# yuw444/fastF

Hardware: AMD Instinct MI355X
Metric: BAM records/sec -> deduped UMI matrix; achieved HBM GB/s vs roofline (higher is better)
Workload: dtype u64

## Files before the change

fastf_amd/csrc/umi_engine.hip:

```cpp
#include "umi_kernels.hpp"
#include "sweep_kernels.hpp"
#include "cap_kernels.hpp"
#include "level_kernels.hpp"
#include "gene_kernels.hpp"
#include "cells_kernels.hpp"
#include "fidelity_kernels.hpp"
#include "gene_fidelity_kernels.hpp"
#include "neighbors_kernels.hpp"
#include "labels_kernels.hpp"

#include <algorithm>
#include <cstdarg>
#include <cstdio>
#include <cstdlib>
#include <cstring>
#include <mutex>
#include <new>
#include <stdexcept>
#include <chrono>
#include <string>
#include <thread>
#include <utility>
#include <vector>

// ... 210 lines not shown
    bool h_coo_pinned = false; u32 h_coo_uses = 0;
    u32* lent_rows = nullptr; u64 lent_cap = 0;
    u32* rows_at = nullptr; u64 rows_stride = 0;
    std::vector<u32> h_ufeature, h_ucell, h_uumi, h_ncopy;
    std::vector<uint8_t> h_unonnull;
    u64 total_records = 0, hits_so_far = 0, keys_so_far = 0;
    u64 c_sampled = 0, c_valid = 0;
    bool finished = false; int sorted_in_tmp = 0; u64 n_sorted = 0;
    u32 skip_bits = 0;
    bool fully_sorted = false;
    DevBuf d_cellidx, d_tilecnt, d_tilebase, d_binbase, d_cnt;
    DevBuf d_halfhits;
    DevBuf d_segkeys;
    DevBuf d_segcount, d_segprefix, d_tileseg;
    u32 giant_parity = 0;
    u32 seg_n = 0; u64 seg_stride = 0;
    DevBuf d_rgn_phys, d_rgn_hist, d_rgn_blk;
    u32 rgn_hist_n = 0, rgn_hist_shift = 0;
    bool stream_mode = false, store_regions = false;
    bool stream_single = false, stream_sharded = false, stream_off = false;
    bool narrow = false, genes_one_family = false;
    u64 slots_used = 0, slot_cap = 0; u32 rgn_n = 0, rgn_cap = 0;
    DevBuf d_scanblk;
    DevBuf d_rg_feature, d_rg_cell, d_rg_count, d_rg_ukeys, d_spanrows, d_spanbase, d_giant;
    u32 rg_n = 0; bool rg_umi = false;
    bool wide = false, long_umi = false; u32 group_bits = 0;
    u32 sub_bits = 0, row_split = 0;
    bool finish_queued = false;
    DevBuf d_vals, d_vtmp;
    bool timing = false;
    hipEvent_t t_ev[2] = {nullptr, nullptr};
    double t_scatter_ms = 0; u64 t_scatter_n = 0;
    double t_k1_ms = 0; u64 t_k1_n = 0;
    double t_k1b_ms = 0; u64 t_k1b_n = 0;
    double t_k3_ms = 0; u64 t_k3_n = 0;
    double t_count_ms = 0; u64 t_count_n = 0;
    double t_gather_ms = 0; u64 t_gather_n = 0;
};
// ... 344 lines not shown
    (void)hipDeviceSynchronize();
    for (int i = 0; i < 2; ++i) {
        fastf_engine::Slot& sl = e->slot[i];
        if (sl.h_stage) (void)hipHostFree(sl.h_stage);
        if (sl.h_draws) (void)hipHostFree(sl.h_draws);
        if (sl.h_small) (void)hipHostFree(sl.h_small);
        sl.d_stage.release();
        if (sl.ev_copy) (void)hipEventDestroy(sl.ev_copy);
        if (sl.ev_done) (void)hipEventDestroy(sl.ev_done);
        if (e->t_ev[i]) (void)hipEventDestroy(e->t_ev[i]);
    }
    if (e->h_small) (void)hipHostFree(e->h_small);
    if (e->h_coo) { if (e->h_coo_pinned) pin_unreg(e->h_coo); fastf_big_free(e->h_coo, (size_t)e->h_coo_cap * 12); }
    e->d_ring.release(); e->d_mt.release(); e->d_nbr.release(); e->d_dbits.release(); e->d_mtwords.release(); e->d_mtsub.release(); e->d_mtpoly.release(); e->d_mtseat.release(); e->d_mtseq.release();
    DevBuf* all[] = {&e->tab_cells, &e->tab_feats, &e->img_cells, &e->img_genes, &e->d_cell_filter, &e->d_keys, &e->d_tmp, &e->d_small, &e->d_feature, &e->d_cell,
                     &e->d_count, &e->d_ukeys, &e->d_ncopy, &e->d_cellidx, &e->d_tilecnt, &e->d_tilebase, &e->d_binbase, &e->d_cnt, &e->d_rg_feature, &e->d_rg_cell, &e->d_rg_count, &e->d_rg_ukeys, &e->d_spanrows, &e->d_spanbase, &e->d_giant, &e->d_scanblk,
                     &e->d_halfhits, &e->d_segcount, &e->d_segprefix, &e->d_tileseg, &e->d_segkeys, &e->d_vals, &e->d_vtmp,
                     &e->d_rgn_phys, &e->d_rgn_hist, &e->d_rgn_blk};
    for (DevBuf* b : all) b->release();
    if (e->s_compute) (void)hipStreamDestroy(e->s_compute);
    if (e->s_copy) (void)hipStreamDestroy(e->s_copy);
    if (e->s_mt) (void)hipStreamDestroy(e->s_mt);
    if (e->ev_mt) (void)hipEventDestroy(e->ev_mt);
    delete e;
} FASTF_CATCH_VOID

extern "C" int fastf_engine_table_modes(const fastf_engine_t* e, int* cells_in_lds, int* genes_in_lds) FASTF_TRY {
    if (!e) return set_err("null engine");
    if (cells_in_lds) *cells_in_lds = e->use_lds_cells;
    if (genes_in_lds) *genes_in_lds = e->use_lds_genes ? (e->lds_genes.direct ? 2 : 1) : 0;
    return 0;
} FASTF_CATCH_INT

// ... 83 lines not shown
    e->t_scatter_n = e->t_k1_n = e->t_k1b_n = e->t_k3_n = e->t_count_n = e->t_gather_n = 0;
    return 0;
} FASTF_CATCH_INT
extern "C" int fastf_engine_get_timing(fastf_engine_t* e, int which, double* total_ms, uint64_t* launches) FASTF_TRY {
    if (!e) return set_err("null engine");
    const double ms[6] = {e->t_k1_ms, e->t_scatter_ms, e->t_k3_ms, e->t_count_ms, e->t_k1b_ms, e->t_gather_ms};
    const u64 n[6] = {e->t_k1_n, e->t_scatter_n, e->t_k3_n, e->t_count_n, e->t_k1b_n, e->t_gather_n};
    if (which < 0 || which > 5) return set_err("bad timer index");
    *total_ms = ms[which]; *launches = n[which];
    return 0;
} FASTF_CATCH_INT

static u64* g_k1_stamps = nullptr;
extern "C" void fastf_debug_set_k1_stamps(void* p) { g_k1_stamps = (u64*)p; }

static void launch_scan_tiles(fastf_engine* e, int slot, hipStream_t s, u32* in, u64* out, u32 T, u64* total_out, u64* running, u64* base_out) {
    constexpr u32 CHUNK = 16u * 1024u;
    const u32 n_blk = (T + CHUNK - 1) / CHUNK;
    if (n_blk <= 1 || n_blk > 64 || e->d_scanblk.ensure(2 * 64 * sizeof(u64))) {
        hipLaunchKernelGGL(scan_tiles_kernel<16>, dim3(1), dim3(1024), 0, s, in, out, T, total_out, running, base_out, (u64*)nullptr);
        return;
    }
    u64* const blk = (u64*)e->d_scanblk.p + 64 * slot;
    hipLaunchKernelGGL(scan_tiles_kernel<16>, dim3(n_blk), dim3(1024), 0, s, in, out, T, (u64*)nullptr, (u64*)nullptr, (u64*)nullptr, blk);
    hipLaunchKernelGGL(scan_fix_kernel<16>, dim3(n_blk), dim3(1024), 0, s, out, T, (const u64*)blk, n_blk, total_out, running, base_out);
}

static int launch_probe_cells(fastf_engine* e, const u64* cb, u64 n, u64* d_total_out, hipStream_t s,
                              u64* d_running = nullptr, u64* d_base_out = nullptr, void* blk = nullptr) {
    if (reserve_workspace(e, blk ? 0 : n, 0, n)) return 1;
    const u32 tiles = (u32)((n + K1_TILE - 1) / K1_TILE);
    const CellOut cout = blk ? CellOut{blk, blk_run_bytes(e->cell16, e->narrow), blk_cell_off(e->narrow)} : CellOut{e->d_cellidx.p, 0u, 0u};
    t_begin(e, s);
    if (e->use_lds_cells) {
        const u32 grid = std::min<u32>(e->cells_blocks_per_cu * g_cu_count, (tiles + 1) / 2);
        if (e->cells_blocks_per_cu >= 2)
            hipLaunchKernelGGL(probe_cells_lds_kernel<true>, dim3(grid), dim3(1024), e->lds_cells.bytes, s, cb, n, e->lds_cells,
                               cout, e->cell16, (u32*)e->d_tilecnt.p, (u32*)e->d_halfhits.p, tiles);
        else
            hipLaunchKernelGGL(probe_cells_lds_kernel<false>, dim3(grid), dim3(1024), e->lds_cells.bytes, s, cb, n, e->lds_cells,
                               cout, e->cell16, (u32*)e->d_tilecnt.p, (u32*)e->d_halfhits.p, tiles);
    } else if (e->cell_filter.bits) {
        const u32 grid = std::min<u32>(tiles, 4 * g_cu_count);
        hipLaunchKernelGGL(probe_cells_filtered_kernel, dim3(grid), dim3(K1_THREADS), (e->cell_filter.mask + 1u) / 8u, s, cb, n,
                           e->cells, e->cell_filter, cout, e->cell16, (u32*)e->d_tilecnt.p, (u32*)e->d_halfhits.p, tiles);
    } else {
        hipLaunchKernelGGL(probe_cells_kernel<0>, dim3(tiles), dim3(K1_THREADS), 0, s, cb, n, e->cells,
                           cout, e->cell16, (u32*)e->d_tilecnt.p, (u32*)e->d_halfhits.p);
    }
    t_end(e, s, &e->t_k1_ms, &e->t_k1_n);
    dbg_sync(s, "K1a probe_cells");
    launch_scan_tiles(e, 0, s, (u32*)e->d_tilecnt.p, (u64*)e->d_tilebase.p, tiles, d_total_out, d_running, d_base_out);
    dbg_sync(s, "K1a tile scan");
    HIP_OK(hipGetLastError());
    return 0;
}

extern "C" int fastf_dev_count_hits(fastf_engine_t* e, const uint64_t* d_cb_key, uint64_t n,
                                    uint64_t* d_hits_out, void* stream) FASTF_TRY {
    DEV_ENTRY(!e, "null engine");
    hipStream_t s = (hipStream_t)stream;
    if (n == 0) { HIP_OK(hipMemsetAsync(d_hits_out, 0, sizeof(u64), s)); return 0; }
    return launch_probe_cells(e, (const u64*)d_cb_key, n, (u64*)d_hits_out, s);
} FASTF_CATCH_INT

extern "C" int fastf_dev_block_bytes(const fastf_engine_t* e, uint64_t n, uint64_t* bytes) FASTF_TRY {
    if (!e || !bytes) return set_err("null argument");
    *bytes = 0;
    if (e->multi || !(e->stream_single || e->stream_sharded) || e->stream_off) return 0;
    *bytes = ((n + BLK_RECS - 1) / BLK_RECS) * (u64)blk_run_bytes(e->cell16, e->narrow);
    return 0;
} FASTF_CATCH_INT

static void launch_block_records(const fastf_engine* e, const u64* gx, const u32* umi, const u32* meta, u64 n, void* blk, hipStream_t s) {
    const u64 units = (n + BLK_RECS - 1) / BLK_RECS;
    const dim3 grid((u32)std::min<u64>((units + 3) / 4, 16ull * g_cu_count));
    if (e->narrow) hipLaunchKernelGGL(block_records_kernel<true>, grid, dim3(256), 0, s, gx, umi, meta, n, (unsigned char*)blk,
                                      blk_run_bytes(e->cell16, true), e->lds_genes.family, e->L);
// ... 622 lines not shown
    if (segmented || stream_shards) {
        u32 grid; u64 region;
        stream_geometry(e, tiles, &grid, &region);
        const u32 n_rgn = grid * (u32)K1S_SUB, rgn0 = app ? app->rgn0 : 0u;
        if (stream_shards) {
            if (e->d_segkeys.ensure((size_t)n_rgn * region * sizeof(u64))) return 1;
            p.keys = (u64*)e->d_segkeys.p;
        } else if ((u64)n_rgn * region > j.stride) return set_err("segmented key output needs %llu slots, the buffer has %llu (fastf_dev_probe_capacity)",
                                                                (unsigned long long)((u64)n_rgn * region), (unsigned long long)j.stride);
        if (app) {
            if (e->rgn_cap < rgn0 + n_rgn) return set_err("internal error: region tables too small");
        } else {
            if (e->rgn_n) return set_err("device-level K1 on an engine that holds pushed chunks: fastf_engine_reset first");
            if (grow_regions(e, n_rgn)) return 1;
        }
        if (e->d_segprefix.ensure(((size_t)n_rgn + 1) * sizeof(u64))) return 1;
        StreamParams sp{(const u32*)e->d_halfhits.p, region, (u64*)e->d_segcount.p + rgn0,
                        stream_shards ? nullptr : (u32*)e->d_rgn_hist.p + (size_t)rgn0 * RADIX, (u64*)e->d_rgn_phys.p + rgn0,
                        app ? app->slot0 : 0ull, e->skip_bits};
        const bool roomy = e->genes_blocks_per_cu < 2;
        const u32 variant = (blk ? (e->narrow ? 16u : 8u) : 0u) | (roomy ? 4u : 0u) | (e->cell16 ? 2u : 0u) | (e->lds_genes.direct ? 1u : 0u);
        hipLaunchKernelGGL(stream_kernel(variant), dim3(grid), dim3(roomy ? K1S_THREADS_ROOMY : K1S_THREADS), e->lds_genes.bytes, s, p, sp);
        if (stream_shards) {
            hipLaunchKernelGGL(shard_partition_kernel, dim3(n_rgn), dim3(SP_THREADS), 0, s, (const u64*)e->d_segkeys.p, (const u64*)e->d_segcount.p,
                               region, e->L.cell_shift, e->n_shards, j.keys, j.stride, j.key_counts, j.counters + 3);
        } else if (app) {
            hipLaunchKernelGGL(seg_scan_kernel, dim3(1), dim3(1024), 0, s, (const u64*)e->d_segcount.p + rgn0, n_rgn, (u64*)e->d_segprefix.p, j.key_counts, true);
        } else {
            hipLaunchKernelGGL(seg_scan_kernel, dim3(1), dim3(1024), 0, s, (const u64*)e->d_segcount.p, n_rgn, (u64*)e->d_segprefix.p, j.key_counts, false);
            e->seg_n = n_rgn; e->seg_stride = region;
            e->rgn_hist_n = n_rgn; e->rgn_hist_shift = e->skip_bits;
        }
    } else if (e->use_lds_genes) {
        const u32 grid = std::min<u32>(tiles, e->genes_blocks_per_cu * g_cu_count);
        if (e->genes_blocks_per_cu >= 2) hipLaunchKernelGGL((filter_pack_kernel<true, false>), dim3(grid), dim3(K1B_THREADS), e->lds_genes.bytes, s, p);
        else hipLaunchKernelGGL((filter_pack_kernel<true, true>), dim3(grid), dim3(K1B_THREADS), e->lds_genes.bytes, s, p);
    } else {
        hipLaunchKernelGGL(filter_pack_kernel<false>, dim3(tiles), dim3(K1B_THREADS), 0, s, p);
    }
    HIP_OK(hipGetLastError());
    t_end(e, s, &e->t_k1b_ms, &e->t_k1b_n);
    dbg_sync(s, blk ? "K1b filter_pack (blocked)" : "K1b filter_pack");
    return 0;
}

// ... 112 lines not shown
    if (max_n == 0) return 0;
    if (max_n >= (1ull << 32)) return set_err("sort of %llu keys: limit is 2^32-1 per shard", (unsigned long long)max_n);
    if (reserve_workspace(e, 0, max_n)) return 1;
    const u32 ipt = choose_sort_ipt(max_n);
    const u32 T = (u32)((max_n + (u64)ipt * SORT_THREADS - 1) / ((u64)ipt * SORT_THREADS));
    u32* bintot = (u32*)e->d_binbase.p; u32* cnt = (u32*)e->d_cnt.p;
    SegMap seg{nullptr, nullptr, 0, 0};
    bool walk = false;
    if (segmented_input) {
        if (!e->seg_n) return set_err("FASTF_SORT_SEGMENTED without a preceding FASTF_PROBE_SEGMENTED probe_pack");
        if (passes == 0) return set_err("segmented keys need at least one sort pass");
        static const bool no_walk = getenv("FASTF_NO_REGION_WALK") != nullptr;
        walk = e->rgn_hist_n == e->seg_n && e->rgn_hist_shift == low_bit && !no_walk && !vals;
        if (!walk) {
            if (!e->seg_stride) return set_err("internal error: regions without a common stride need their histograms");
            seg = SegMap{(const u64*)e->d_segprefix.p, (const TileSeg*)e->d_tileseg.p, e->seg_n, e->seg_stride};
            hipLaunchKernelGGL(seg_tiles_kernel, dim3(std::min<u32>((T + 255) / 256, 1024)), dim3(256), 0, s, seg.prefix, seg.n_seg,
                               seg.stride, ipt * SORT_THREADS, (TileSeg*)e->d_tileseg.p);
        }
    }
    const SegMap none{nullptr, nullptr, 0, 0};
    for (u32 q = 0; q < passes; ++q) {
        const u64* src = (q & 1) ? tmp : keys;
        u64* dst = (q & 1) ? keys : tmp;
        const u32 shift = low_bit + 8 * q;
        if (q == 0 && walk) {
            const u32 R = e->seg_n, n_blk = (R + RGN_BLK - 1) / RGN_BLK;
            if (e->d_rgn_blk.ensure((size_t)n_blk * RADIX * sizeof(u32))) return 1;
            hipLaunchKernelGGL(rgn_scan_blocks_kernel, dim3(n_blk), dim3(RADIX), 0, s, (u32*)e->d_rgn_hist.p, R, (u32*)e->d_rgn_blk.p);
            hipLaunchKernelGGL(rgn_scan_fix_kernel, dim3(n_blk), dim3(RADIX), 0, s, (u32*)e->d_rgn_hist.p, R, (const u32*)e->d_rgn_blk.p, n_blk, bintot);
            t_begin(e, s);
            hipLaunchKernelGGL(scatter_regions_kernel, dim3(tile_grid(R)), dim3(SORT_THREADS), scatter_smem_bytes(ipt), s, src, dst,
                               (const u64*)e->d_rgn_phys.p, (const u64*)e->d_segcount.p, (const u32*)e->d_rgn_hist.p, (const u32*)bintot, R, ipt, shift,
                               max_n >= (24ull << 20));
            t_end(e, s, &e->t_scatter_ms, &e->t_scatter_n);
            e->rgn_hist_n = 0;
            dbg_sync(s, "K2 sort pass (region walk)");
            continue;
        }
        t_begin(e, s);
        if (q == 0 && seg.prefix) hipLaunchKernelGGL(tile_count_kernel<true>, dim3(tile_grid(T)), dim3(SORT_THREADS), 0, s, src, d_n, shift, cnt, ipt, seg);
        else hipLaunchKernelGGL(tile_count_kernel<false>, dim3(tile_grid(T)), dim3(SORT_THREADS), 0, s, src, d_n, shift, cnt, ipt, none);
        t_end(e, s, &e->t_count_ms, &e->t_count_n);
        hipLaunchKernelGGL(row_scan_kernel, dim3(RADIX), dim3(1024), 0, s, cnt, d_n, bintot, ipt);
        t_begin(e, s);
        if (vals) launch_scatter(shift, T, s, src, dst, d_n, (const u32*)cnt, (const u32*)bintot, ipt, none, (q & 1) ? vtmp : vals, (q & 1) ? vals : vtmp);
        else launch_scatter(shift, T, s, src, dst, d_n, (const u32*)cnt, (const u32*)bintot, ipt, q == 0 ? seg : none);
        t_end(e, s, &e->t_scatter_ms, &e->t_scatter_n);
        dbg_sync(s, "K2 sort pass");
    }
    HIP_OK(hipGetLastError());
    return 0;
}

extern "C" int fastf_dev_set_regions(fastf_engine_t* e, const uint64_t* d_counts, uint32_t n_regions, uint64_t stride,
                                     uint64_t* d_n_out, void* stream) FASTF_TRY {
    DEV_SINGLE(!e || !d_counts || !d_n_out, "null argument");
    if (n_regions == 0 || stride == 0) return set_err("fastf_dev_set_regions: no regions");
    HIP_OK(hipSetDevice(e->device));
    if (e->d_segprefix.ensure(((size_t)n_regions + 1) * sizeof(u64))) return 1;
    hipLaunchKernelGGL(seg_scan_kernel, dim3(1), dim3(1024), 0, (hipStream_t)stream, (const u64*)d_counts, (u32)n_regions, (u64*)e->d_segprefix.p, (u64*)d_n_out);
    HIP_OK(hipGetLastError());
    e->seg_n = n_regions; e->seg_stride = stride; e->rgn_hist_n = 0;
    return 0;
} FASTF_CATCH_INT

extern "C" int fastf_dev_sort(fastf_engine_t* e, uint64_t* d_keys, uint64_t* d_tmp, const uint64_t* d_n,
                              uint64_t max_n, uint32_t key_bits, uint32_t flags, int* sorted_in_tmp, void* stream) FASTF_TRY {
    DEV_SINGLE(!e, "null engine");
    NO_WIDE(e, "fastf_dev_sort");
    HIP_OK(hipSetDevice(e->device));
    int dummy = 0;
    return launch_sort(e, (u64*)d_keys, (u64*)d_tmp, (const u64*)d_n, max_n, key_bits,
                       (flags & FASTF_SORT_SKIP_LOW) ? e->skip_bits : 0,
                       sorted_in_tmp ? sorted_in_tmp : &dummy, (hipStream_t)stream, (flags & FASTF_SORT_SEGMENTED) != 0);
} FASTF_CATCH_INT

static u32 k3_grid(u64 max_n, int dedup) {
// ... 682 lines not shown
    u64 nrows = 0;
    uk.clear(); uv.clear(); e->h_ncopy.clear();
    if (!n) return 0;
    u64 *kc = e->sorted_in_tmp ? (u64*)e->d_tmp.p : (u64*)e->d_keys.p, *ko = e->sorted_in_tmp ? (u64*)e->d_keys.p : (u64*)e->d_tmp.p;
    u64 *vc = e->sorted_in_tmp ? (u64*)e->d_vtmp.p : (u64*)e->d_vals.p, *vo = e->sorted_in_tmp ? (u64*)e->d_vals.p : (u64*)e->d_vtmp.p;
    if (!e->fully_sorted) {
        int f = 0;
        if (launch_sort(e, vc, vo, small + SM_KEYCOUNT, n, e->L.feat_shift, 0, &f, s, false, kc, ko)) return 1;
        if (f) { std::swap(kc, ko); std::swap(vc, vo); }
        if (launch_sort(e, kc, ko, small + SM_KEYCOUNT, n, e->group_bits, 0, &f, s, false, vc, vo)) return 1;
        if (f) { std::swap(kc, ko); std::swap(vc, vo); }
        e->sorted_in_tmp = kc == (u64*)e->d_tmp.p;
        e->fully_sorted = true;
    }
    const u64 T = (n + UW_TILE - 1) / UW_TILE;
    if (e->d_ukeys.ensure(n * 8) || e->d_ncopy.ensure(n * 4) || e->d_rg_ukeys.ensure(2 * n * 8) || e->d_scanblk.ensure(2 * 64 * sizeof(u64))) return 1;
    DevBuf cnt, base;
    if (cnt.ensure((T + 16) * 4) || base.ensure((T + 16) * 8)) { cnt.release(); base.release(); return 1; }
    int rc = 0;
    do {
        if (hipMemsetAsync(cnt.p, 0, (T + 16) * 4, s) != hipSuccess) { rc = set_err("memset failed"); break; }
        const u32 grid = (u32)std::min<u64>(T, 16ull * g_cu_count);
        hipLaunchKernelGGL(pair_heads_kernel, dim3(grid), dim3(UW_THREADS), 0, s, (const u64*)kc, (const u64*)vc, (const u64*)(small + SM_KEYCOUNT), (u32*)cnt.p);
        launch_scan_tiles(e, 1, s, (u32*)cnt.p, (u64*)base.p, (u32)T, small + SM_NROWS_U, nullptr, nullptr);
        u64* uvals = (u64*)e->d_rg_ukeys.p; u64* hpos = uvals + n;
        hipLaunchKernelGGL(pair_rows_kernel, dim3(grid), dim3(UW_THREADS), 0, s, (const u64*)kc, (const u64*)vc, (const u64*)(small + SM_KEYCOUNT),
                           (const u64*)base.p, (u64*)e->d_ukeys.p, uvals, hpos);
        hipLaunchKernelGGL(pair_copies_kernel, dim3(grid), dim3(UW_THREADS), 0, s, (const u64*)hpos, (const u64*)(small + SM_NROWS_U),
                           (const u64*)(small + SM_KEYCOUNT), (u32*)e->d_ncopy.p);
        if (hipGetLastError() != hipSuccess) { rc = set_err("kernel launch failed (distinct pairs of wide keys)"); break; }
        if (hipMemcpyAsync(e->h_small, small, SM_WORDS * sizeof(u64), hipMemcpyDeviceToHost, s) != hipSuccess || hipStreamSynchronize(s) != hipSuccess) { rc = set_err("device error in the distinct pairs of wide keys"); break; }
        if (e->h_small[SM_COUNTERS + 3]) { rc = set_err("%s", err_bits_text(e->h_small[SM_COUNTERS + 3])); break; }
        nrows = e->h_small[SM_NROWS_U];
        if (nrows > n) { rc = set_err("internal error: %llu distinct pairs out of %llu keys", (unsigned long long)nrows, (unsigned long long)n); break; }
        uk.resize(nrows); uv.resize(nrows); e->h_ncopy.resize(nrows);
        if (nrows) {
            if (copy_d2h(uk.data(), e->d_ukeys.p, nrows * 8) || copy_d2h(uv.data(), uvals, nrows * 8) || copy_d2h(e->h_ncopy.data(), e->d_ncopy.p, nrows * 4)) { rc = 1; break; }
        }
    } while (0);
// ... 168 lines not shown
```

fastf_amd/csrc/umi_kernels.hpp:

```cpp
#pragma once
#if !defined(FASTF_EXPERIMENT)
#  if defined(FASTF_X_ANY)
#    error "FASTF_X_* knobs need -DFASTF_EXPERIMENT (experiment builds only: tools/build_variant.sh)"
#  endif
#endif
#ifndef FASTF_K1_IPT
#define FASTF_K1_IPT 8
#endif
#ifndef FASTF_K1_THREADS
#define FASTF_K1_THREADS 512
#endif
#include <hip/hip_runtime.h>
#include <stdint.h>
#include <type_traits>

namespace fastf {

typedef unsigned long long u64;
typedef unsigned int u32;

constexpr int WAVE = 64;

constexpr u64 ERR_DRAWS_SHORT  = 2;
constexpr u64 ERR_UMI_TOOLONG  = 4;
// ... 363 lines not shown
        const i32x4_t v = __builtin_amdgcn_raw_buffer_load_b128(rsrc, (int)(h[j] * 16u), 0, AUX);
        s[j] = make_uint4((u32)v[0], (u32)v[1], (u32)v[2], (u32)v[3]);
    }
#pragma unroll
    for (int j = 0; j < N; ++j) {
        const u64 k = ((u64)s[j].y << 32) | s[j].x;
        u32 v = 0;
        if (key[j] != 0) {
            if (k == key[j]) v = s[j].z;
            else if (k != 0) v = table_probe_from(t, key[j], (h[j] + 1) & t.mask);
        }
        val[j] = v;
    }
}

template <u32 PER>
__global__ __launch_bounds__(1024) void scan_tiles_kernel(u32* __restrict__ in, u64* __restrict__ out, u32 T,
                                                          u64* __restrict__ total_out, u64* __restrict__ running = nullptr,
                                                          u64* __restrict__ base_out = nullptr, u64* __restrict__ blk_tot = nullptr) {
    __shared__ u32 s_w[16];
    __shared__ u64 s_carry;
    const int lane = lane_id(), w = threadIdx.x >> 6;
    if (threadIdx.x == 0) s_carry = 0;
    __syncthreads();
    const u32 t_first = blk_tot ? blockIdx.x * PER * 1024u : 0u, t_end = blk_tot ? (t_first + PER * 1024u < T ? t_first + PER * 1024u : T) : T;
    for (u32 t0 = t_first; t0 < t_end; t0 += PER * 1024) {
        const u32 t = t0 + PER * threadIdx.x;
        u32 v[PER];
        if (t + PER <= T) {
#pragma unroll
            for (u32 q = 0; q < PER / 4; ++q) {
                const uint4 x = reinterpret_cast<const uint4*>(in + t)[q];
                v[4 * q] = x.x; v[4 * q + 1] = x.y; v[4 * q + 2] = x.z; v[4 * q + 3] = x.w;
                reinterpret_cast<uint4*>(in + t)[q] = make_uint4(0, 0, 0, 0);
            }
        } else {
#pragma unroll
            for (u32 k = 0; k < PER; ++k) { v[k] = t + k < T ? in[t + k] : 0; if (t + k < T) in[t + k] = 0; }
        }
        u32 sum = 0;
#pragma unroll
        for (u32 k = 0; k < PER; ++k) sum += v[k];
        const u32 inc = wave_incl_scan32(sum, lane);
        if (lane == WAVE - 1) s_w[w] = inc;
        __syncthreads();
        u64 off = s_carry;
        for (int i = 0; i < w; ++i) off += s_w[i];
        u64 e = off + inc - sum;
        if (t + PER <= T) {
#pragma unroll
            for (u32 q = 0; q < PER / 2; ++q) {
                reinterpret_cast<ulonglong2*>(out + t)[q] = make_ulonglong2(e, e + v[2 * q]);
                e += (u64)v[2 * q] + v[2 * q + 1];
            }
        } else {
#pragma unroll
            for (u32 k = 0; k < PER; ++k) { if (t + k < T) out[t + k] = e; e += v[k]; }
        }
        __syncthreads();
        if (threadIdx.x == 1023) s_carry = off + inc;
        __syncthreads();
    }
    if (blk_tot) { if (threadIdx.x == 0) blk_tot[blockIdx.x] = s_carry; return; }
    if (threadIdx.x == 0 && total_out) *total_out = s_carry;
    if (threadIdx.x == 0 && running) { const u64 r = *running; *base_out = r; *running = r + s_carry; }
}

template <u32 PER>
__global__ __launch_bounds__(1024) void scan_fix_kernel(u64* __restrict__ out, u32 T, const u64* __restrict__ blk_tot, u32 n_blk,
                                                        u64* __restrict__ total_out, u64* __restrict__ running, u64* __restrict__ base_out) {
    u64 off = 0, total = 0;
    for (u32 i = 0; i < n_blk; ++i) { const u64 v = blk_tot[i]; if (i < blockIdx.x) off += v; total += v; }
    if (blockIdx.x == 0 && threadIdx.x == 0) {
        if (total_out) *total_out = total;
        if (running) { const u64 r = *running; *base_out = r; *running = r + total; }
    }
    if (blockIdx.x == 0 || off == 0) return;
    const u32 t_first = blockIdx.x * PER * 1024u;
    for (u32 k = threadIdx.x; k < PER * 1024u && t_first + k < T; k += 1024) out[t_first + k] += off;
}

constexpr int K1_THREADS = FASTF_K1_THREADS, K1_IPT = FASTF_K1_IPT, K1_TILE = K1_THREADS * K1_IPT, K1_WAVES = K1_THREADS / WAVE;
static_assert(K1_THREADS == 512 && K1_IPT == 8, "K1a layout: 8 waves x 8 items x 64 lanes per tile");

constexpr u32 BLK_RECS = 256, BLK_GX = 0, BLK_UMI = 2048, BLK_META = 3072, BLK_CELL = 4096;
constexpr u32 NBLK_GX = 0, NBLK_UM = 1024, NBLK_CELL = 2048;
__host__ __device__ __forceinline__ u32 blk_cell_off(bool narrow) { return narrow ? NBLK_CELL : BLK_CELL; }
__host__ __device__ __forceinline__ u32 blk_run_bytes(bool c16, bool narrow = false) { return blk_cell_off(narrow) + (c16 ? 2u : 4u) * BLK_RECS; }
struct CellOut { void* p; u32 run; u32 off; };
__device__ __forceinline__ void put_cell(const CellOut o, bool c16, u64 idx, u32 v) {
    unsigned char* at = reinterpret_cast<unsigned char*>(o.p);
    u64 i = idx;
    if (o.run) { at += (idx / BLK_RECS) * o.run + o.off; i = idx % BLK_RECS; }
    if (c16) reinterpret_cast<unsigned short*>(at)[i] = (unsigned short)v; else reinterpret_cast<u32*>(at)[i] = v;
// ... 673 lines not shown
    {
        u32 e = errs;
#pragma unroll
        for (int o = 32; o > 0; o >>= 1) e |= __shfl_xor(e, o, WAVE);
        if (lane == 0 && e) atomicOr(&s_err, e);
    }
    __syncthreads();
    const int te = w * WAVE + lane;
    if (te < 3 && s_tot[te]) atomicAdd(&p.counters[te], s_tot[te]);
    if (te == 3 && s_err) atomicOr(&p.counters[3], (u64)s_err);
    if (te >= 64 && te < 64 + K1S_SUB) {
        const u32 r = blockIdx.x * K1S_SUB + (u32)(te - 64);
        sp.seg_count[r] = s_cursor[te - 64];
        if (sp.rgn_hist) sp.rgn_phys[r] = sp.slot0 + (u64)r * sp.region_stride;
    }
    if (sp.rgn_hist)
        for (int i = te; i < K1S_SUB * K1S_BINS; i += THREADS) sp.rgn_hist[(u64)blockIdx.x * (K1S_SUB * K1S_BINS) + i] = s_hist[i];
}

template <bool NARROW>
__global__ __launch_bounds__(256) void block_records_kernel(const u64* __restrict__ gx, const u32* __restrict__ umi, const u32* __restrict__ meta,
                                                            u64 n, unsigned char* __restrict__ blk, u32 run, u32 family, const KeyLayout L) {
    const u64 units = (n + BLK_RECS - 1) / BLK_RECS, waves = (u64)gridDim.x * (blockDim.x / WAVE);
    const int lane = lane_id();
    for (u64 u = (u64)blockIdx.x * (blockDim.x / WAVE) + (threadIdx.x >> 6); u < units; u += waves) {
        unsigned char* const r = blk + u * run;
#pragma unroll
        for (int j = 0; j < (int)BLK_RECS / WAVE; ++j) {
            const u32 o = (u32)j * WAVE + (u32)lane;
            const u64 i = u * BLK_RECS + o;
// ... 374 lines not shown
#endif
        if (tile >= T) return;
        const u64 base = (u64)tile * tile_keys;
        const u32 n_valid = (u32)((n - base) < (u64)tile_keys ? (n - base) : (u64)tile_keys);
        int tid = (int)threadIdx.x;
        asm volatile("" : "+v"(tid));
        const u32 g_off = tid < RADIX ? off[(u64)tid * row_stride(T) + tile] : 0u;
        if (n_valid == tile_keys) (void)scatter_tile<SHIFT, true, SEG, VALS>(in, out, base, n_valid, tile, g_off, bin_tot, (int)ipt, smem, rshift, seg, tid, streams, stamps, vin, vout);
        else (void)scatter_tile<SHIFT, false, SEG, VALS>(in, out, base, n_valid, tile, g_off, bin_tot, (int)ipt, smem, rshift, seg, tid, streams, stamps, vin, vout);
        if constexpr (VALS) __syncthreads();
    }
}

constexpr u32 RGN_BLK = 64;
static_assert(K1S_BINS == RADIX, "K1b's region histograms are histograms of a sort digit");
__global__ __launch_bounds__(RADIX) void rgn_scan_blocks_kernel(u32* __restrict__ hist, u32 R, u32* __restrict__ blk_sum) {
    const u32 d = threadIdx.x, r0 = blockIdx.x * RGN_BLK, r1 = r0 + RGN_BLK < R ? r0 + RGN_BLK : R;
    u32 acc = 0;
    for (u32 r = r0; r < r1; r += 8) {
        u32 v[8];
#pragma unroll
        for (u32 k = 0; k < 8; ++k) v[k] = r + k < r1 ? hist[(u64)(r + k) * RADIX + d] : 0u;
#pragma unroll
        for (u32 k = 0; k < 8; ++k) { if (r + k < r1) hist[(u64)(r + k) * RADIX + d] = acc; acc += v[k]; }
    }
    blk_sum[(u64)blockIdx.x * RADIX + d] = acc;
}
__global__ __launch_bounds__(RADIX) void rgn_scan_fix_kernel(u32* __restrict__ hist, u32 R, const u32* __restrict__ blk_sum, u32 n_blk,
                                                             u32* __restrict__ bin_tot) {
    const u32 d = threadIdx.x, w = blockIdx.x;
    u32 off = 0, tot = 0;
    for (u32 i = 0; i < n_blk; ++i) { const u32 v = blk_sum[(u64)i * RADIX + d]; off += i < w ? v : 0u; tot += v; }
    if (w == 0) bin_tot[d] = tot;
    if (off == 0) return;
    const u32 r0 = w * RGN_BLK, r1 = r0 + RGN_BLK < R ? r0 + RGN_BLK : R;
    for (u32 r = r0; r < r1; ++r) hist[(u64)r * RADIX + d] += off;
}
__global__ __launch_bounds__(SORT_THREADS, 8) void scatter_regions_kernel(const u64* __restrict__ keys, u64* __restrict__ out,
                                                                           const u64* __restrict__ rgn_phys, const u64* __restrict__ rgn_count,
                                                                           const u32* __restrict__ hist_excl, const u32* __restrict__ bin_tot,
                                                                           u32 R, u32 ipt, u32 rshift, bool streams) {
    extern __shared__ __attribute__((aligned(16))) unsigned char smem[];
    const u32 tile_keys = ipt * SORT_THREADS;
    const SegMap none{nullptr, nullptr, 0, 0};
    for (u32 i = blockIdx.x >> 3;; i += gridDim.x >> 3) {
        const u32 r = xcd_tile(R, i);
        if (r >= R) return;
        const u64 cnt = rgn_count[r];
        const u64* const in = keys + rgn_phys[r];
        u32 acc = threadIdx.x < RADIX ? hist_excl[(u64)r * RADIX + threadIdx.x] : 0u;
        for (u64 base = 0; base < cnt; base += tile_keys) {
// ... 682 lines not shown
```

Before: 112.3 billion.

## Collapse multi-launch scans into single-pass kernels and defer segment prefix scan

Replaces the two-kernel tile scan (block scan plus fix-up) with one single-block kernel that scans twelve rows per round using a two-level wave scan. It also replaces the two-kernel region histogram scan with one kernel that recomputes each block's front sum by reading all earlier rows, writing offsets to a separate buffer. The segment prefix scan in the non-append K1 path is deferred until the sort actually needs it, and the key count is accumulated by atomics in the K1 kernel instead. The aim is fewer launches and dependent serial steps. The cost is redundant reads of earlier histogram rows, which grow quadratically with region count, and a single block doing the whole tile scan serially.

Result: no change. 111.7 billion (-0.5%).

```diff
diff --git a/fastf_amd/csrc/umi_engine.hip b/fastf_amd/csrc/umi_engine.hip
--- a/fastf_amd/csrc/umi_engine.hip
+++ b/fastf_amd/csrc/umi_engine.hip
@@ -248,14 +248,14 @@
     DevBuf d_segkeys;
     DevBuf d_segcount, d_segprefix, d_tileseg;
     u32 giant_parity = 0;
+    bool seg_prefix_ok = false;
     u32 seg_n = 0; u64 seg_stride = 0;
-    DevBuf d_rgn_phys, d_rgn_hist, d_rgn_blk;
+    DevBuf d_rgn_phys, d_rgn_hist, d_rgn_off;
     u32 rgn_hist_n = 0, rgn_hist_shift = 0;
     bool stream_mode = false, store_regions = false;
     bool stream_single = false, stream_sharded = false, stream_off = false;
     bool narrow = false, genes_one_family = false;
     u64 slots_used = 0, slot_cap = 0; u32 rgn_n = 0, rgn_cap = 0;
-    DevBuf d_scanblk;
     DevBuf d_rg_feature, d_rg_cell, d_rg_count, d_rg_ukeys, d_spanrows, d_spanbase, d_giant;
     u32 rg_n = 0; bool rg_umi = false;
     bool wide = false, long_umi = false; u32 group_bits = 0;
@@ -630,9 +630,9 @@
     if (e->h_coo) { if (e->h_coo_pinned) pin_unreg(e->h_coo); fastf_big_free(e->h_coo, (size_t)e->h_coo_cap * 12); }
     e->d_ring.release(); e->d_mt.release(); e->d_nbr.release(); e->d_dbits.release(); e->d_mtwords.release(); e->d_mtsub.release(); e->d_mtpoly.release(); e->d_mtseat.release(); e->d_mtseq.release();
     DevBuf* all[] = {&e->tab_cells, &e->tab_feats, &e->img_cells, &e->img_genes, &e->d_cell_filter, &e->d_keys, &e->d_tmp, &e->d_small, &e->d_feature, &e->d_cell,
-                     &e->d_count, &e->d_ukeys, &e->d_ncopy, &e->d_cellidx, &e->d_tilecnt, &e->d_tilebase, &e->d_binbase, &e->d_cnt, &e->d_rg_feature, &e->d_rg_cell, &e->d_rg_count, &e->d_rg_ukeys, &e->d_spanrows, &e->d_spanbase, &e->d_giant, &e->d_scanblk,
+                     &e->d_count, &e->d_ukeys, &e->d_ncopy, &e->d_cellidx, &e->d_tilecnt, &e->d_tilebase, &e->d_binbase, &e->d_cnt, &e->d_rg_feature, &e->d_rg_cell, &e->d_rg_count, &e->d_rg_ukeys, &e->d_spanrows, &e->d_spanbase, &e->d_giant,
                      &e->d_halfhits, &e->d_segcount, &e->d_segprefix, &e->d_tileseg, &e->d_segkeys, &e->d_vals, &e->d_vtmp,
-                     &e->d_rgn_phys, &e->d_rgn_hist, &e->d_rgn_blk};
+                     &e->d_rgn_phys, &e->d_rgn_hist, &e->d_rgn_off};
     for (DevBuf* b : all) b->release();
     if (e->s_compute) (void)hipStreamDestroy(e->s_compute);
     if (e->s_copy) (void)hipStreamDestroy(e->s_copy);
@@ -746,16 +746,8 @@
 static u64* g_k1_stamps = nullptr;
 extern "C" void fastf_debug_set_k1_stamps(void* p) { g_k1_stamps = (u64*)p; }
 
-static void launch_scan_tiles(fastf_engine* e, int slot, hipStream_t s, u32* in, u64* out, u32 T, u64* total_out, u64* running, u64* base_out) {
-    constexpr u32 CHUNK = 16u * 1024u;
-    const u32 n_blk = (T + CHUNK - 1) / CHUNK;
-    if (n_blk <= 1 || n_blk > 64 || e->d_scanblk.ensure(2 * 64 * sizeof(u64))) {
-        hipLaunchKernelGGL(scan_tiles_kernel<16>, dim3(1), dim3(1024), 0, s, in, out, T, total_out, running, base_out, (u64*)nullptr);
-        return;
-    }
-    u64* const blk = (u64*)e->d_scanblk.p + 64 * slot;
-    hipLaunchKernelGGL(scan_tiles_kernel<16>, dim3(n_blk), dim3(1024), 0, s, in, out, T, (u64*)nullptr, (u64*)nullptr, (u64*)nullptr, blk);
-    hipLaunchKernelGGL(scan_fix_kernel<16>, dim3(n_blk), dim3(1024), 0, s, out, T, (const u64*)blk, n_blk, total_out, running, base_out);
+static void launch_scan_tiles(hipStream_t s, u32* in, u64* out, u32 T, u64* total_out, u64* running, u64* base_out) {
+    hipLaunchKernelGGL(scan_tiles_kernel, dim3(1), dim3(1024), 0, s, in, out, T, total_out, running, base_out);
 }
 
 static int launch_probe_cells(fastf_engine* e, const u64* cb, u64 n, u64* d_total_out, hipStream_t s,
@@ -782,7 +774,7 @@
     }
     t_end(e, s, &e->t_k1_ms, &e->t_k1_n);
     dbg_sync(s, "K1a probe_cells");
-    launch_scan_tiles(e, 0, s, (u32*)e->d_tilecnt.p, (u64*)e->d_tilebase.p, tiles, d_total_out, d_running, d_base_out);
+    launch_scan_tiles(s, (u32*)e->d_tilecnt.p, (u64*)e->d_tilebase.p, tiles, d_total_out, d_running, d_base_out);
     dbg_sync(s, "K1a tile scan");
     HIP_OK(hipGetLastError());
     return 0;
@@ -794,6 +786,33 @@
     hipStream_t s = (hipStream_t)stream;
     if (n == 0) { HIP_OK(hipMemsetAsync(d_hits_out, 0, sizeof(u64), s)); return 0; }
     return launch_probe_cells(e, (const u64*)d_cb_key, n, (u64*)d_hits_out, s);
+} FASTF_CATCH_INT
+
+extern "C" int fastf_debug_tile_scan(fastf_engine_t* e, const uint64_t* d_cb_key, uint64_t n, uint64_t* d_total_out, uint64_t* d_running,
+                                     uint64_t* d_base_out, uint64_t* h_tile_base, uint32_t* h_tile_hits, void* stream) FASTF_TRY {
+    DEV_ENTRY(!e || !h_tile_base || !h_tile_hits, "null argument");
+    if (n == 0 || (d_running != nullptr) != (d_base_out != nullptr)) return set_err("fastf_debug_tile_scan: no records, or one of running / base without the other");
+    hipStream_t s = (hipStream_t)stream;
+    if (launch_probe_cells(e, (const u64*)d_cb_key, n, (u64*)d_total_out, s, (u64*)d_running, (u64*)d_base_out)) return 1;
+    HIP_OK(hipStreamSynchronize(s));
+    const size_t tiles = (size_t)((n + K1_TILE - 1) / K1_TILE);
+    return copy_d2h(h_tile_base, e->d_tilebase.p, tiles * sizeof(u64)) || copy_d2h(h_tile_hits, e->d_tilecnt.p, tiles * sizeof(u32));
+} FASTF_CATCH_INT
+
+extern "C" uint32_t fastf_debug_regions(const fastf_engine_t* e) { return e && !e->multi ? e->seg_n : 0u; }
+extern "C" int fastf_debug_region_offsets(fastf_engine_t* e, const uint32_t* h_hist, uint32_t R, uint32_t* h_offs, uint32_t* h_bin_tot) FASTF_TRY {
+    DEV_ENTRY(!e || !h_hist || !h_offs || !h_bin_tot, "null argument");
+    if (R == 0) return set_err("fastf_debug_region_offsets: no regions");
+    const size_t bytes = (size_t)R * RADIX * sizeof(u32);
+    DevBuf hist, offs, tot;
+    int rc = hist.ensure(bytes) || offs.ensure(bytes) || tot.ensure(RADIX * sizeof(u32)) || copy_h2d(hist.p, h_hist, bytes);
+    if (!rc) {
+        hipLaunchKernelGGL(rgn_offsets_kernel, dim3((R + RGN_BLK - 1) / RGN_BLK), dim3(RGN_OFF_THREADS), 0, (hipStream_t)0, (const u32*)hist.p, R, (u32*)offs.p, (u32*)tot.p);
+        rc = hipGetLastError() != hipSuccess || hipDeviceSynchronize() != hipSuccess ? set_err("rgn_offsets_kernel failed") : 0;
+    }
+    if (!rc) rc = copy_d2h(h_offs, offs.p, bytes) || copy_d2h(h_bin_tot, tot.p, RADIX * sizeof(u32));
+    hist.release(); offs.release(); tot.release();
+    return rc;
 } FASTF_CATCH_INT
 
 extern "C" int fastf_dev_block_bytes(const fastf_engine_t* e, uint64_t n, uint64_t* bytes) FASTF_TRY {
@@ -1446,7 +1465,8 @@
             if (e->rgn_n) return set_err("device-level K1 on an engine that holds pushed chunks: fastf_engine_reset first");
             if (grow_regions(e, n_rgn)) return 1;
         }
-        if (e->d_segprefix.ensure(((size_t)n_rgn + 1) * sizeof(u64))) return 1;
+        p.key_counts = segmented && !app ? j.key_counts : nullptr;
+        if (app && e->d_segprefix.ensure(((size_t)n_rgn + 1) * sizeof(u64))) return 1;
         StreamParams sp{(const u32*)e->d_halfhits.p, region, (u64*)e->d_segcount.p + rgn0,
                         stream_shards ? nullptr : (u32*)e->d_rgn_hist.p + (size_t)rgn0 * RADIX, (u64*)e->d_rgn_phys.p + rgn0,
                         app ? app->slot0 : 0ull, e->skip_bits};
@@ -1459,8 +1479,7 @@
         } else if (app) {
             hipLaunchKernelGGL(seg_scan_kernel, dim3(1), dim3(1024), 0, s, (const u64*)e->d_segcount.p + rgn0, n_rgn, (u64*)e->d_segprefix.p, j.key_counts, true);
         } else {
-            hipLaunchKernelGGL(seg_scan_kernel, dim3(1), dim3(1024), 0, s, (const u64*)e->d_segcount.p, n_rgn, (u64*)e->d_segprefix.p, j.key_counts, false);
-            e->seg_n = n_rgn; e->seg_stride = region;
+            e->seg_n = n_rgn; e->seg_stride = region; e->seg_prefix_ok = false;
             e->rgn_hist_n = n_rgn; e->rgn_hist_shift = e->skip_bits;
         }
     } else if (e->use_lds_genes) {
@@ -1603,6 +1622,12 @@
         walk = e->rgn_hist_n == e->seg_n && e->rgn_hist_shift == low_bit && !no_walk && !vals;
         if (!walk) {
             if (!e->seg_stride) return set_err("internal error: regions without a common stride need their histograms");
+            if (!e->seg_prefix_ok) {
+                if (e->d_segprefix.ensure(((size_t)e->seg_n + 2) * sizeof(u64))) return 1;
+                hipLaunchKernelGGL(seg_scan_kernel, dim3(1), dim3(1024), 0, s, (const u64*)e->d_segcount.p, e->seg_n, (u64*)e->d_segprefix.p,
+                                   (u64*)e->d_segprefix.p + e->seg_n + 1, false);
+                e->seg_prefix_ok = true;
+            }
             seg = SegMap{(const u64*)e->d_segprefix.p, (const TileSeg*)e->d_tileseg.p, e->seg_n, e->seg_stride};
             hipLaunchKernelGGL(seg_tiles_kernel, dim3(std::min<u32>((T + 255) / 256, 1024)), dim3(256), 0, s, seg.prefix, seg.n_seg,
                                seg.stride, ipt * SORT_THREADS, (TileSeg*)e->d_tileseg.p);
@@ -1615,12 +1640,11 @@
         const u32 shift = low_bit + 8 * q;
         if (q == 0 && walk) {
             const u32 R = e->seg_n, n_blk = (R + RGN_BLK - 1) / RGN_BLK;
-            if (e->d_rgn_blk.ensure((size_t)n_blk * RADIX * sizeof(u32))) return 1;
-            hipLaunchKernelGGL(rgn_scan_blocks_kernel, dim3(n_blk), dim3(RADIX), 0, s, (u32*)e->d_rgn_hist.p, R, (u32*)e->d_rgn_blk.p);
-            hipLaunchKernelGGL(rgn_scan_fix_kernel, dim3(n_blk), dim3(RADIX), 0, s, (u32*)e->d_rgn_hist.p, R, (const u32*)e->d_rgn_blk.p, n_blk, bintot);
+            if (e->d_rgn_off.ensure((size_t)R * RADIX * sizeof(u32))) return 1;
+            hipLaunchKernelGGL(rgn_offsets_kernel, dim3(n_blk), dim3(RGN_OFF_THREADS), 0, s, (const u32*)e->d_rgn_hist.p, R, (u32*)e->d_rgn_off.p, bintot);
             t_begin(e, s);
             hipLaunchKernelGGL(scatter_regions_kernel, dim3(tile_grid(R)), dim3(SORT_THREADS), scatter_smem_bytes(ipt), s, src, dst,
-                               (const u64*)e->d_rgn_phys.p, (const u64*)e->d_segcount.p, (const u32*)e->d_rgn_hist.p, (const u32*)bintot, R, ipt, shift,
+                               (const u64*)e->d_rgn_phys.p, (const u64*)e->d_segcount.p, (const u32*)e->d_rgn_off.p, (const u32*)bintot, R, ipt, shift,
                                max_n >= (24ull << 20));
             t_end(e, s, &e->t_scatter_ms, &e->t_scatter_n);
             e->rgn_hist_n = 0;
@@ -1650,7 +1674,7 @@
     if (e->d_segprefix.ensure(((size_t)n_regions + 1) * sizeof(u64))) return 1;
     hipLaunchKernelGGL(seg_scan_kernel, dim3(1), dim3(1024), 0, (hipStream_t)stream, (const u64*)d_counts, (u32)n_regions, (u64*)e->d_segprefix.p, (u64*)d_n_out);
     HIP_OK(hipGetLastError());
-    e->seg_n = n_regions; e->seg_stride = stride; e->rgn_hist_n = 0;
+    e->seg_n = n_regions; e->seg_stride = stride; e->rgn_hist_n = 0; e->seg_prefix_ok = true;
     return 0;
 } FASTF_CATCH_INT
 
@@ -2363,7 +2387,7 @@
         e->fully_sorted = true;
     }
     const u64 T = (n + UW_TILE - 1) / UW_TILE;
-    if (e->d_ukeys.ensure(n * 8) || e->d_ncopy.ensure(n * 4) || e->d_rg_ukeys.ensure(2 * n * 8) || e->d_scanblk.ensure(2 * 64 * sizeof(u64))) return 1;
+    if (e->d_ukeys.ensure(n * 8) || e->d_ncopy.ensure(n * 4) || e->d_rg_ukeys.ensure(2 * n * 8)) return 1;
     DevBuf cnt, base;
     if (cnt.ensure((T + 16) * 4) || base.ensure((T + 16) * 8)) { cnt.release(); base.release(); return 1; }
     int rc = 0;
@@ -2371,7 +2395,7 @@
         if (hipMemsetAsync(cnt.p, 0, (T + 16) * 4, s) != hipSuccess) { rc = set_err("memset failed"); break; }
         const u32 grid = (u32)std::min<u64>(T, 16ull * g_cu_count);
         hipLaunchKernelGGL(pair_heads_kernel, dim3(grid), dim3(UW_THREADS), 0, s, (const u64*)kc, (const u64*)vc, (const u64*)(small + SM_KEYCOUNT), (u32*)cnt.p);
-        launch_scan_tiles(e, 1, s, (u32*)cnt.p, (u64*)base.p, (u32)T, small + SM_NROWS_U, nullptr, nullptr);
+        launch_scan_tiles(s, (u32*)cnt.p, (u64*)base.p, (u32)T, small + SM_NROWS_U, nullptr, nullptr);
         u64* uvals = (u64*)e->d_rg_ukeys.p; u64* hpos = uvals + n;
         hipLaunchKernelGGL(pair_rows_kernel, dim3(grid), dim3(UW_THREADS), 0, s, (const u64*)kc, (const u64*)vc, (const u64*)(small + SM_KEYCOUNT),
                            (const u64*)base.p, (u64*)e->d_ukeys.p, uvals, hpos);
diff --git a/fastf_amd/csrc/umi_kernels.hpp b/fastf_amd/csrc/umi_kernels.hpp
--- a/fastf_amd/csrc/umi_kernels.hpp
+++ b/fastf_amd/csrc/umi_kernels.hpp
@@ -401,70 +401,70 @@
     }
 }
 
-template <u32 PER>
+constexpr u32 SCAN_Q = 12, SCAN_ROW = 4 * 1024, SCAN_ROUND = SCAN_Q * SCAN_ROW;
 __global__ __launch_bounds__(1024) void scan_tiles_kernel(u32* __restrict__ in, u64* __restrict__ out, u32 T,
                                                           u64* __restrict__ total_out, u64* __restrict__ running = nullptr,
-                                                          u64* __restrict__ base_out = nullptr, u64* __restrict__ blk_tot = nullptr) {
-    __shared__ u32 s_w[16];
+                                                          u64* __restrict__ base_out = nullptr) {
+    static_assert(SCAN_Q * 16 == 3 * WAVE, "wave 0 scans the wave totals of a round three to a lane");
+    __shared__ u32 s_w[SCAN_Q * 16];
+    __shared__ u32 s_round;
     __shared__ u64 s_carry;
     const int lane = lane_id(), w = threadIdx.x >> 6;
     if (threadIdx.x == 0) s_carry = 0;
-    __syncthreads();
-    const u32 t_first = blk_tot ? blockIdx.x * PER * 1024u : 0u, t_end = blk_tot ? (t_first + PER * 1024u < T ? t_first + PER * 1024u : T) : T;
-    for (u32 t0 = t_first; t0 < t_end; t0 += PER * 1024) {
-        const u32 t = t0 + PER * threadIdx.x;
-        u32 v[PER];
-        if (t + PER <= T) {
-#pragma unroll
-            for (u32 q = 0; q < PER / 4; ++q) {
-                const uint4 x = reinterpret_cast<const uint4*>(in + t)[q];
-                v[4 * q] = x.x; v[4 * q + 1] = x.y; v[4 * q + 2] = x.z; v[4 * q + 3] = x.w;
-                reinterpret_cast<uint4*>(in + t)[q] = make_uint4(0, 0, 0, 0);
-            }
-        } else {
-#pragma unroll
-            for (u32 k = 0; k < PER; ++k) { v[k] = t + k < T ? in[t + k] : 0; if (t + k < T) in[t + k] = 0; }
-        }
-        u32 sum = 0;
-#pragma unroll
-        for (u32 k = 0; k < PER; ++k) sum += v[k];
-        const u32 inc = wave_incl_scan32(sum, lane);
-        if (lane == WAVE - 1) s_w[w] = inc;
-        __syncthreads();
-        u64 off = s_carry;
-        for (int i = 0; i < w; ++i) off += s_w[i];
-        u64 e = off + inc - sum;
-        if (t + PER <= T) {
-#pragma unroll
-            for (u32 q = 0; q < PER / 2; ++q) {
-                reinterpret_cast<ulonglong2*>(out + t)[q] = make_ulonglong2(e, e + v[2 * q]);
-                e += (u64)v[2 * q] + v[2 * q + 1];
-            }
-        } else {
-#pragma unroll
-            for (u32 k = 0; k < PER; ++k) { if (t + k < T) out[t + k] = e; e += v[k]; }
-        }
-        __syncthreads();
-        if (threadIdx.x == 1023) s_carry = off + inc;
-        __syncthreads();
-    }
-    if (blk_tot) { if (threadIdx.x == 0) blk_tot[blockIdx.x] = s_carry; return; }
-    if (threadIdx.x == 0 && total_out) *total_out = s_carry;
-    if (threadIdx.x == 0 && running) { const u64 r = *running; *base_out = r; *running = r + s_carry; }
-}
-
-template <u32 PER>
-__global__ __launch_bounds__(1024) void scan_fix_kernel(u64* __restrict__ out, u32 T, const u64* __restrict__ blk_tot, u32 n_blk,
-                                                        u64* __restrict__ total_out, u64* __restrict__ running, u64* __restrict__ base_out) {
-    u64 off = 0, total = 0;
-    for (u32 i = 0; i < n_blk; ++i) { const u64 v = blk_tot[i]; if (i < blockIdx.x) off += v; total += v; }
-    if (blockIdx.x == 0 && threadIdx.x == 0) {
+    for (u32 t0 = 0; t0 < T; t0 += SCAN_ROUND) {
+        uint4 v[SCAN_Q];
+        u32 inc[SCAN_Q];
+#pragma unroll
+        for (u32 q = 0; q < SCAN_Q; ++q) {
+            const u32 t = t0 + q * SCAN_ROW + 4 * threadIdx.x;
+            v[q] = make_uint4(0, 0, 0, 0);
+            if (t < T) {
+                if (T - t >= 4) {
+                    v[q] = *reinterpret_cast<const uint4*>(in + t);
+                    *reinterpret_cast<uint4*>(in + t) = make_uint4(0, 0, 0, 0);
+                } else {
+                    v[q].x = in[t]; in[t] = 0;
+                    if (T - t > 1) { v[q].y = in[t + 1]; in[t + 1] = 0; }
+                    if (T - t > 2) { v[q].z = in[t + 2]; in[t + 2] = 0; }
+                }
+            }
+        }
+#pragma unroll
+        for (u32 q = 0; q < SCAN_Q; ++q) {
+            inc[q] = wave_incl_scan32(v[q].x + v[q].y + v[q].z + v[q].w, lane);
+            if (lane == WAVE - 1) s_w[q * 16 + w] = inc[q];
+        }
+        __syncthreads();
+        if (w == 0) {
+            const u32 a = s_w[3 * lane], b = s_w[3 * lane + 1], c = s_w[3 * lane + 2];
+            const u32 i3 = wave_incl_scan32(a + b + c, lane), e3 = i3 - (a + b + c);
+            s_w[3 * lane] = e3; s_w[3 * lane + 1] = e3 + a; s_w[3 * lane + 2] = e3 + a + b;
+            if (lane == WAVE - 1) s_round = i3;
+        }
+        __syncthreads();
+        const u64 carry = s_carry;
+#pragma unroll
+        for (u32 q = 0; q < SCAN_Q; ++q) {
+            const u32 t = t0 + q * SCAN_ROW + 4 * threadIdx.x;
+            if (t >= T) continue;
+            const u64 e = carry + s_w[q * 16 + w] + (inc[q] - (v[q].x + v[q].y + v[q].z + v[q].w));
+            if (T - t >= 4) {
+                reinterpret_cast<ulonglong2*>(out + t)[0] = make_ulonglong2(e, e + v[q].x);
+                reinterpret_cast<ulonglong2*>(out + t)[1] = make_ulonglong2(e + v[q].x + v[q].y, e + v[q].x + v[q].y + v[q].z);
+            } else {
+                out[t] = e;
+                if (T - t > 1) out[t + 1] = e + v[q].x;
+                if (T - t > 2) out[t + 2] = e + v[q].x + v[q].y;
+            }
+        }
+        __syncthreads();
+        if (threadIdx.x == 0) s_carry = carry + s_round;
+    }
+    if (threadIdx.x == 0) {
+        const u64 total = s_carry;
         if (total_out) *total_out = total;
         if (running) { const u64 r = *running; *base_out = r; *running = r + total; }
     }
-    if (blockIdx.x == 0 || off == 0) return;
-    const u32 t_first = blockIdx.x * PER * 1024u;
-    for (u32 k = threadIdx.x; k < PER * 1024u && t_first + k < T; k += 1024) out[t_first + k] += off;
 }
 
 constexpr int K1_THREADS = FASTF_K1_THREADS, K1_IPT = FASTF_K1_IPT, K1_TILE = K1_THREADS * K1_IPT, K1_WAVES = K1_THREADS / WAVE;
@@ -1168,6 +1168,12 @@
         sp.seg_count[r] = s_cursor[te - 64];
         if (sp.rgn_hist) sp.rgn_phys[r] = sp.slot0 + (u64)r * sp.region_stride;
     }
+    if (te == 64 + K1S_SUB && p.key_counts) {
+        u64 c = 0;
+#pragma unroll
+        for (int i = 0; i < K1S_SUB; ++i) c += s_cursor[i];
+        if (c) atomicAdd(&p.key_counts[0], c);
+    }
     if (sp.rgn_hist)
         for (int i = te; i < K1S_SUB * K1S_BINS; i += THREADS) sp.rgn_hist[(u64)blockIdx.x * (K1S_SUB * K1S_BINS) + i] = s_hist[i];
 }
@@ -1572,27 +1578,46 @@
 
 constexpr u32 RGN_BLK = 64;
 static_assert(K1S_BINS == RADIX, "K1b's region histograms are histograms of a sort digit");
-__global__ __launch_bounds__(RADIX) void rgn_scan_blocks_kernel(u32* __restrict__ hist, u32 R, u32* __restrict__ blk_sum) {
-    const u32 d = threadIdx.x, r0 = blockIdx.x * RGN_BLK, r1 = r0 + RGN_BLK < R ? r0 + RGN_BLK : R;
-    u32 acc = 0;
-    for (u32 r = r0; r < r1; r += 8) {
-        u32 v[8];
-#pragma unroll
-        for (u32 k = 0; k < 8; ++k) v[k] = r + k < r1 ? hist[(u64)(r + k) * RADIX + d] : 0u;
-#pragma unroll
-        for (u32 k = 0; k < 8; ++k) { if (r + k < r1) hist[(u64)(r + k) * RADIX + d] = acc; acc += v[k]; }
-    }
-    blk_sum[(u64)blockIdx.x * RADIX + d] = acc;
-}
-__global__ __launch_bounds__(RADIX) void rgn_scan_fix_kernel(u32* __restrict__ hist, u32 R, const u32* __restrict__ blk_sum, u32 n_blk,
-                                                             u32* __restrict__ bin_tot) {
-    const u32 d = threadIdx.x, w = blockIdx.x;
-    u32 off = 0, tot = 0;
-    for (u32 i = 0; i < n_blk; ++i) { const u32 v = blk_sum[(u64)i * RADIX + d]; off += i < w ? v : 0u; tot += v; }
-    if (w == 0) bin_tot[d] = tot;
-    if (off == 0) return;
-    const u32 r0 = w * RGN_BLK, r1 = r0 + RGN_BLK < R ? r0 + RGN_BLK : R;
-    for (u32 r = r0; r < r1; ++r) hist[(u64)r * RADIX + d] += off;
+constexpr u32 RGN_OFF_THREADS = 1024, RGN_OFF_WAVES = RGN_OFF_THREADS / WAVE, RGN_OWN = RGN_BLK / RGN_OFF_WAVES;
+static_assert(RADIX == 4 * WAVE && RGN_BLK % RGN_OFF_WAVES == 0, "a wave covers a histogram row, four digits to a lane");
+__device__ __forceinline__ uint4 add4(uint4 a, uint4 b) { return make_uint4(a.x + b.x, a.y + b.y, a.z + b.z, a.w + b.w); }
+__global__ __launch_bounds__(RGN_OFF_THREADS) void rgn_offsets_kernel(const u32* __restrict__ hist, u32 R, u32* __restrict__ offs,
+                                                                      u32* __restrict__ bin_tot) {
+    __shared__ uint4 s_front[RGN_OFF_WAVES][WAVE], s_own[RGN_OFF_WAVES][WAVE];
+    const u32 lane = threadIdx.x & (WAVE - 1), g = threadIdx.x >> 6;
+    const u32 r0 = blockIdx.x * RGN_BLK;
+    const uint4* const rows = reinterpret_cast<const uint4*>(hist);
+    uint4 own[RGN_OWN];
+#pragma unroll
+    for (u32 k = 0; k < RGN_OWN; ++k) {
+        const u32 r = r0 + g * RGN_OWN + k;
+        own[k] = r < R ? rows[(u64)r * WAVE + lane] : make_uint4(0, 0, 0, 0);
+    }
+    uint4 front = make_uint4(0, 0, 0, 0);
+    for (u32 r = g; r < r0; r += 8 * RGN_OFF_WAVES) {
+        uint4 x[8];
+#pragma unroll
+        for (u32 k = 0; k < 8; ++k) x[k] = r + k * RGN_OFF_WAVES < r0 ? rows[(u64)(r + k * RGN_OFF_WAVES) * WAVE + lane] : make_uint4(0, 0, 0, 0);
+#pragma unroll
+        for (u32 k = 0; k < 8; ++k) front = add4(front, x[k]);
+    }
+    uint4 mine = own[0];
+#pragma unroll
+    for (u32 k = 1; k < RGN_OWN; ++k) mine = add4(mine, own[k]);
+    s_front[g][lane] = front; s_own[g][lane] = mine;
+    __syncthreads();
+    uint4 acc = make_uint4(0, 0, 0, 0);
+#pragma unroll
+    for (u32 i = 0; i < RGN_OFF_WAVES; ++i) acc = add4(acc, s_front[i][lane]);
+    for (u32 i = 0; i < g; ++i) acc = add4(acc, s_own[i][lane]);
+    uint4* const dst = reinterpret_cast<uint4*>(offs);
+#pragma unroll
+    for (u32 k = 0; k < RGN_OWN; ++k) {
+        const u32 r = r0 + g * RGN_OWN + k;
+        if (r < R) dst[(u64)r * WAVE + lane] = acc;
+        acc = add4(acc, own[k]);
+    }
+    if (blockIdx.x == gridDim.x - 1 && g == RGN_OFF_WAVES - 1) reinterpret_cast<uint4*>(bin_tot)[lane] = acc;
 }
 __global__ __launch_bounds__(SORT_THREADS, 8) void scatter_regions_kernel(const u64* __restrict__ keys, u64* __restrict__ out,
                                                                            const u64* __restrict__ rgn_phys, const u64* __restrict__ rgn_count,
```
